# lia2790/walking-controllers

Measured on AMD Instinct MI355X. Metric: QP solves/sec (whole node), iCub IK-QP + DCM-MPC batch at 1/2/4/8 MI355X, higher is better.
Workload: dtype f64

## Files before the change

walking-controllers_amd/csrc/ik4.hip:

```cpp
#include "ik4_device.h"

namespace {

template <bool TICK, int JSRC, bool LOG = false, bool EXT = false>
__global__ __launch_bounds__(64, WCQP_IK4_WAVES)
void ik4_kernel(const IkDeviceParams* __restrict__ prm, int batch,
                const double* __restrict__ JL, const double* __restrict__ JR,
                const double* __restrict__ JN, const double* __restrict__ JC,
                const double* qpos, const double* __restrict__ state,
                double* __restrict__ dq_out, int* __restrict__ status_out,
                unsigned* __restrict__ alo_out, unsigned* __restrict__ aup_out,
                double* __restrict__ ferr_out, int* __restrict__ iters_out, const wcqp_tick::TickDev* __restrict__ tdp, int phase, int n_inner, int skip_last_mpc)
{
    __shared__ __attribute__((aligned(16))) double smem[4][PER_INST];
    if constexpr (TICK) {
        __shared__ __attribute__((aligned(16))) double kmodel[JSRC == 2 ? wcqp_tick::kKinTabSize : 2];
        __shared__ __attribute__((aligned(16))) double kgains[JSRC == 2 ? 4 * wcqp_tick::kGainsLdsStages : 2];
        ik4_tick_walk<JSRC, LOG, EXT, false>(prm, batch, JL, JR, JN, JC, qpos, state, dq_out, status_out, alo_out, aup_out, ferr_out, iters_out,
                                             tdp, phase, n_inner, skip_last_mpc, smem, kmodel, kgains);
    } else {
        ik4_body<TICK, JSRC>(prm, batch, JL, JR, JN, JC, qpos, state, dq_out, status_out, alo_out, aup_out, ferr_out, iters_out, wcqp_tick::TickDev{}, smem, xcd_group((int)blockIdx.x, (int)gridDim.x));
    }
}

// ... 1 lines not shown
__global__ __launch_bounds__(64)
void tick_mpc_prime_kernel(wcqp_tick::TickDev td, int t)
{
    __shared__ __attribute__((aligned(16))) double s_hull[4][WCQP_HULL_ROWS][4];
    const int lane = threadIdx.x, grp = lane >> 4, j = lane & 15;
    const long inst_raw = (long)blockIdx.x * 4 + grp;
    const bool live = inst_raw < td.batch;
    const long inst = live ? inst_raw : (long)td.batch - 1;
    wcqp_tick::TickMpcRegs mreg;
    wcqp_tick::tick_mpc_issue(td, j, inst, t, mreg);
    wcqp_tick::tick_mpc_finish<false, EXT>(td, j, inst, live, t, mreg, s_hull[grp]);
}


__global__ __launch_bounds__(64, WCQP_IK4_WAVES)
void qp_pair_kernel(const IkDeviceParams* __restrict__ prm, int batch,
                    const double* __restrict__ JL, const double* __restrict__ JR,
                    const double* __restrict__ JN, const double* __restrict__ JC,
                    const double* qpos, const double* __restrict__ state,
                    double* __restrict__ dq_out, int* __restrict__ status_out,
                    unsigned* __restrict__ alo_out, unsigned* __restrict__ aup_out,
                    double* __restrict__ ferr_out, int* __restrict__ iters_out, int ik_blocks, MpcPairArgs m)
{
    __shared__ __attribute__((aligned(16))) double smem[4][PER_INST];
    const bool is_mpc = (int)blockIdx.x >= ik_blocks;
    const int blk = is_mpc ? (int)blockIdx.x - ik_blocks : xcd_group((int)blockIdx.x, ik_blocks);
    if (is_mpc) {
        static_assert(wcqp_mpc::kInstPerWave * WCQP_HULL_ROWS * 4 <= 4 * PER_INST, "the hull rows fit the IK's LDS");
        double (*s_hull)[WCQP_HULL_ROWS][4] = reinterpret_cast<double (*)[WCQP_HULL_ROWS][4]>(&smem[0][0]);
        const int lane = threadIdx.x;
        const int sub = lane / wcqp_mpc::kLanesPerInstance, t = lane % wcqp_mpc::kLanesPerInstance;
        const long inst_raw = (long)blk * wcqp_mpc::kInstPerWave + sub;
        const bool live = inst_raw < batch;
        const long inst = live ? inst_raw : (long)batch - 1;
        const double2* rp = reinterpret_cast<const double2*>(m.ref) + inst * m.ref_len;
        double ux, uy, margin;
        int st;
        unsigned mask;
        wcqp_mpc::mpc_row_solve(m.c, t, inst, m.x0, rp, m.ref_len, m.u_prev, m.hull_A, m.hull_b, m.hull_nc, inst, s_hull[sub], ux, uy, st, mask, margin);
        if (t == 0 && live) {
            reinterpret_cast<double2*>(m.u0)[inst] = make_double2(ux, uy);
            m.status[inst] = st;
            if (m.active) m.active[inst] = mask;
            if (m.margin) m.margin[inst] = margin;
        }
        return;
    }
    ik4_body<false>(prm, batch, JL, JR, JN, JC, qpos, state, dq_out, status_out, alo_out, aup_out, ferr_out, iters_out, wcqp_tick::TickDev{}, smem, blk);
}

template <bool WITH_MPC>
__device__ __forceinline__
void plan_walk(const IkDeviceParams* __restrict__ prm, int batch, const wcqp_qp_step* __restrict__ recs, int n_steps, int ways, int groups,
               const wcqp_mpc::MpcDeviceConsts& c, unsigned* queue, double (*smem)[PER_INST])
{
    const bool dynamic = ways == 0;
    unsigned z = threadIdx.x;
    __asm__ volatile("" : "+v"(z));
    z >>= 6;
    constexpr unsigned QS = wcqp_ik::kPlanQueueStride / 4u;
    const unsigned total = (unsigned)n_steps * (unsigned)groups;
    unsigned home = blockIdx.x % wcqp_ik::kPlanQueues;
    auto draw = [&]() -> unsigned {
#ifndef WCQP_PLAN_STEAL
#define WCQP_PLAN_STEAL (wcqp_ik::kPlanQueues - 1u)
#endif
        for (unsigned tried = 0; tried <= WCQP_PLAN_STEAL; ++tried) {
            unsigned k = 0;
            if (threadIdx.x == 0) k = __hip_atomic_fetch_add(queue + home * QS + z, 1u, __ATOMIC_RELAXED, __HIP_MEMORY_SCOPE_AGENT);
            const unsigned u = (unsigned)__builtin_amdgcn_readfirstlane((int)k) * wcqp_ik::kPlanQueues + home;
            if (u < total) return u;
            home = (home + 1u) % wcqp_ik::kPlanQueues;
        }
        return total;
    };
    int r = (int)blockIdx.x / groups, blk = (int)blockIdx.x % groups;
#ifndef WCQP_PLAN_NO_XCD_MAP
    if ((groups & 7) == 0) {
        const int n = groups >> 3, x = (int)blockIdx.x & 7, k = (int)blockIdx.x >> 3;
        r = k / n; blk = x * n + k % n;
    }
#endif
    if (dynamic) {
        const unsigned u = draw();
        r = u < total ? (int)(u % (unsigned)n_steps) : n_steps; blk = u < total ? (int)(u / (unsigned)n_steps) : 0;
    }
#pragma unroll 1
    while (r < n_steps) {
        __asm__ volatile("" ::: "memory");
        using wcqp::as_global;
        const wcqp_qp_step& s = recs[r];
        MpcPairArgs m{c, WITH_MPC ? as_global(s.x0) : nullptr, WITH_MPC ? as_global(s.ref) : nullptr, s.ref_len, WITH_MPC ? as_global(s.u_prev) : nullptr,
                      WITH_MPC ? as_global(s.hull_A) : nullptr, WITH_MPC ? as_global(s.hull_b) : nullptr, WITH_MPC ? as_global(s.hull_nc) : nullptr,
                      WITH_MPC ? as_global(s.u0) : nullptr, WITH_MPC ? as_global(s.mpc_status) : nullptr, WITH_MPC ? as_global(s.mpc_active) : nullptr,
                      WITH_MPC ? as_global(s.mpc_margin) : nullptr,
                      dynamic ? queue + home * QS + z : nullptr, 0u, WITH_MPC};
        ik4_body<false, 0, true>(prm, batch, as_global(s.J_left), as_global(s.J_right), as_global(s.J_neck), as_global(s.J_com), as_global(s.q), as_global(s.state),
                                 as_global(s.dq), as_global(s.ik_status), as_global(s.active_lower), as_global(s.active_upper),
                                 as_global(s.foot_err), as_global(s.iters), wcqp_tick::TickDev{}, smem, blk, 0, true, nullptr, nullptr, &m);
        wcqp::wave_lds_fence();
        if (dynamic) {
            unsigned u = (unsigned)__builtin_amdgcn_readfirstlane((int)m.ticket) * wcqp_ik::kPlanQueues + home;
            if (u >= total) { home = (home + 1u) % wcqp_ik::kPlanQueues; u = draw(); }
            r = u < total ? (int)(u % (unsigned)n_steps) : n_steps; blk = u < total ? (int)(u / (unsigned)n_steps) : 0;
        } else {
            r += ways;
        }
    }
    if (dynamic && threadIdx.x == 0) {
        __threadfence();
        if (atomicAdd(queue + wcqp_ik::kPlanQueues * QS, 1u) == gridDim.x - 1) {
            for (unsigned q = 0; q <= wcqp_ik::kPlanQueues; ++q) queue[q * QS] = 0u;
        }
    }
}

__global__ __launch_bounds__(64, WCQP_IK4_WAVES)
void qp_plan_kernel(const IkDeviceParams* __restrict__ prm, int batch, const wcqp_qp_step* __restrict__ recs, int n_steps, int ways, int groups,
                    wcqp_mpc::MpcDeviceConsts c, unsigned* queue)
{
    __shared__ __attribute__((aligned(16))) double smem[4][PER_INST];
    plan_walk<true>(prm, batch, recs, n_steps, ways, groups, c, queue, smem);
}
__global__ __launch_bounds__(64, WCQP_IK4_WAVES) WCQP_IK_PLAN_REGS
void ik_plan_kernel(const IkDeviceParams* __restrict__ prm, int batch, const wcqp_qp_step* __restrict__ recs, int n_steps, int ways, int groups,
                    wcqp_mpc::MpcDeviceConsts c, unsigned* queue)
{
    __shared__ __attribute__((aligned(16))) double smem[4][PER_INST];
    plan_walk<false>(prm, batch, recs, n_steps, ways, groups, c, queue, smem);
}

}

namespace wcqp_ik {

int ik4_plan_queue_grid(int batch, int n_steps) {
    int dev = 0, cus = 0;
    if (hipGetDevice(&dev) != hipSuccess || hipDeviceGetAttribute(&cus, hipDeviceAttributeMultiprocessorCount, dev) != hipSuccess || cus < 1) return -1;
    const long long total = (long long)((batch + 3) / 4) * n_steps, slots = (long long)cus * 4 * WCQP_IK4_WAVES;
    return (int)(total < slots ? total : slots);
}

int ik4_launch_plan(const IkDeviceParams* d_prm, int batch, const wcqp_qp_step* d_recs, int n_steps, int ways,
                    const wcqp_mpc::MpcDeviceConsts& c, hipStream_t stream, unsigned* d_queue, int queue_grid, bool ik_only) {
    if (!d_prm || !d_recs || batch < 1 || n_steps < 1 || ways < 0 || (ways == 0 && (!d_queue || queue_grid < 1))) return WCQP_E_INVALID;
    const int groups = (batch + 3) / 4;
    if ((long long)groups * n_steps >= (1ll << 31)) return WCQP_E_INVALID;
    const unsigned grid = ways == 0 ? (unsigned)queue_grid : (unsigned)(groups * ways);
    if (ik_only) hipLaunchKernelGGL(ik_plan_kernel, dim3(grid), dim3(64), 0, stream, d_prm, batch, d_recs, n_steps, ways, groups, c, d_queue);
    else hipLaunchKernelGGL(qp_plan_kernel, dim3(grid), dim3(64), 0, stream, d_prm, batch, d_recs, n_steps, ways, groups, c, d_queue);
    WCQP_HIP_TRY(hipGetLastError());
    return WCQP_OK;
}

int ik4_launch_pair(const IkDeviceParams* d_prm, int batch, const IkIo& io,
                    const wcqp_mpc::MpcDeviceConsts& c, const double* x0, const double* ref, int ref_len, const double* u_prev,
                    const double* hull_A, const double* hull_b, const int* hull_nc,
                    double* u0, int* mstatus, unsigned* mactive, double* mmargin, hipStream_t stream) {
    const int ik_blocks = (batch + 3) / 4;
    const int mpc_blocks = (batch + wcqp_mpc::kInstPerWave - 1) / wcqp_mpc::kInstPerWave;
    MpcPairArgs m{c, x0, ref, ref_len, u_prev, hull_A, hull_b, hull_nc, u0, mstatus, mactive, mmargin};
    hipLaunchKernelGGL(qp_pair_kernel, dim3((unsigned)(ik_blocks + mpc_blocks)), dim3(64), 0, stream, d_prm, batch,
                       io.JL, io.JR, io.JN, io.JC, io.q, io.state, io.dq, io.status, io.alo, io.aup, io.ferr, io.iters, ik_blocks, m);
    WCQP_HIP_TRY(hipGetLastError());
    return WCQP_OK;
}

template <bool TICK, int JSRC, bool LOG = false, bool EXT = false>
static void ik4_launch_as(const IkDeviceParams* prm, int batch, const IkIo& io, const wcqp_tick::TickDev* td_dev, int phase,
                          int n_inner, int skip_last_mpc, hipStream_t stream) {
    hipLaunchKernelGGL((ik4_kernel<TICK, JSRC, LOG, EXT>), dim3((unsigned)((batch + 3) / 4)), dim3(64), 0, stream, prm, batch,
                       io.JL, io.JR, io.JN, io.JC, io.q, io.state, io.dq, io.status, io.alo, io.aup, io.ferr, io.iters,
                       td_dev, phase, n_inner, skip_last_mpc);
}

int ik4_launch(const IkDeviceParams* d_prm, int batch, const IkIo& io, hipStream_t stream) {
    ik4_launch_as<false, 0>(d_prm, batch, io, nullptr, 0, 1, 0, stream);
    WCQP_HIP_TRY(hipGetLastError());
    return WCQP_OK;
}

static int tick_check(const wcqp_tick::TickDevPL& td, const TickVariant& v) {
// ... 38 lines not shown
```

walking-controllers_amd/csrc/ik4_device.h:

```cpp
#pragma once
#include <cmath>
#include <limits>
#include <type_traits>
#include "ik_common.h"
#include "tick_device.h"
#include "kin_device.h"

namespace {

using namespace wcqp_ik;

typedef double v4d __attribute__((ext_vector_type(4)));

constexpr int NR = 12;
constexpr int NROWS_IN = 18;
constexpr int KMAX = kDof - 9;
constexpr int LDC = 14;

constexpr int OFF_ST = 0;
constexpr int OFF_BV = 112;
constexpr int OFF_DB = 130;
constexpr int OFF_CT = 0;
constexpr int OFF_PB = 0;
constexpr int A_SIZE = 340;
constexpr int OFF_COL = A_SIZE;
constexpr int OFF_YV = A_SIZE + 32;
constexpr int OFF_DV = A_SIZE + 48;
constexpr int OFF_YPV = A_SIZE;
constexpr int OFF_RV = A_SIZE + 16;
constexpr int OFF_CV = A_SIZE + 32;
constexpr int OFF_ROWB = A_SIZE + 48;
constexpr int PER_INST = 440;
constexpr int K_FS = 14, K_TW = 0, K_FRB = 322, K_FR = 358;
constexpr int K_MS = 394, K_MH = 410;
constexpr int K_PF = 434;
__host__ __device__ constexpr int k_sd(int m) { return K_TW + (16 + (m >> 1)) * K_FS + 12 + (m & 1); }
static_assert(K_MH + 24 <= K_PF && K_PF < PER_INST, "the flags stash is clear of the others");
static_assert(kDof * K_FS <= K_FRB && K_FR + 36 <= K_MS && K_MH + 24 <= PER_INST && k_sd(11) < kDof * K_FS && k_sd(0) >= 32 * 4, "kinematics scratch fits; the prefix sums [32][4] stay clear of the anchor pose");
static_assert(OFF_CT + 24 * LDC + 2 <= A_SIZE && OFF_DB + 18 <= A_SIZE && OFF_PB + 12 * 18 <= A_SIZE, "LDS overlays");
static_assert(OFF_ROWB + 16 <= PER_INST && OFF_DV + 16 <= PER_INST && (PER_INST % 32 == 24 || PER_INST % 32 == 8), "instances 16 banks apart");
static_assert(KMAX <= 24, "one slot index per C^T row");
static_assert(PER_INST * 8 * 4 * 11 <= 160 * 1024, "11 blocks per CU");

#ifndef WCQP_IK4_WAVES
#define WCQP_IK4_WAVES 2
#endif
#ifdef WCQP_IK_PLAN_VGPR_HALF
#define WCQP_IK_PLAN_REGS __attribute__((amdgpu_num_vgpr(WCQP_IK_PLAN_VGPR_HALF)))
#else
#define WCQP_IK_PLAN_REGS
#endif
#ifndef WCQP_IK4_KS
#define WCQP_IK4_KS 4
#endif

#if defined(WCQP_TICK_KSTAMPS)
#define WCQP_STAMP_AT(k) do { if constexpr (TICK) { unsigned long long t__; asm volatile("s_memtime %0\n\ts_waitcnt lgkmcnt(0)" : "=s"(t__) :: "memory"); \
                              if (lane == 0 && td.stamps) td.stamps[(size_t)blk * 16 + (k)] = t__; } } while (0)
#define WCQP_STAMP(k) do { if constexpr ((k) == 0 || (k) == 12 || (k) == 14) WCQP_STAMP_AT(k); } while (0)
#define WCQP_KSTAMP(k) WCQP_STAMP_AT(k)
#elif defined(WCQP_TICK_STAMPS)
#define WCQP_STAMP(k) do { if constexpr (TICK) { unsigned long long t__; asm volatile("s_memtime %0\n\ts_waitcnt lgkmcnt(0)" : "=s"(t__) :: "memory"); \
                           if (lane == 0 && td.stamps) td.stamps[(size_t)blk * 16 + (k)] = t__; } } while (0)
#elif defined(WCQP_IK_STAMPS)
#define WCQP_STAMP(k) do { unsigned long long t__; asm volatile("s_memtime %0\n\ts_waitcnt lgkmcnt(0)" : "=s"(t__) :: "memory"); \
                           if (lane == __ffsll((long long)__ballot(true)) - 1) reinterpret_cast<unsigned long long*>(ferr_out)[(size_t)blockIdx.x * 16 + (k)] = t__; } while (0)
#else
#define WCQP_STAMP(k) do { } while (0)
#endif
#ifndef WCQP_KSTAMP
#define WCQP_KSTAMP(k) do { } while (0)
#endif

__device__ __forceinline__ void swap32(double& a, double& b) {
    const auto l = __builtin_amdgcn_permlane32_swap((unsigned)__double2loint(a), (unsigned)__double2loint(b), false, false);
    const auto h = __builtin_amdgcn_permlane32_swap((unsigned)__double2hiint(a), (unsigned)__double2hiint(b), false, false);
    a = __hiloint2double((int)h[0], (int)l[0]); b = __hiloint2double((int)h[1], (int)l[1]);
}
__device__ __forceinline__ void swap16(double& a, double& b) {
    const auto l = __builtin_amdgcn_permlane16_swap((unsigned)__double2loint(a), (unsigned)__double2loint(b), false, false);
    const auto h = __builtin_amdgcn_permlane16_swap((unsigned)__double2hiint(a), (unsigned)__double2hiint(b), false, false);
    a = __hiloint2double((int)h[0], (int)l[0]); b = __hiloint2double((int)h[1], (int)l[1]);
}

using wcqp_kin::st2;
using wcqp_kin::ld2;

struct MpcPairArgs {
    wcqp_mpc::MpcDeviceConsts c;
    const double* x0; const double* ref; int ref_len; const double* u_prev;
    const double* hull_A; const double* hull_b; const int* hull_nc;
    double* u0; int* status; unsigned* active; double* margin;
    unsigned* ticket_from = nullptr; unsigned ticket = 0;
    bool has_mpc = true;
};

template <bool TICK, int JSRC = 0, bool PAIR = false, bool LOG = false, bool EXT = false, bool REACT = false, bool GS = false, bool PL = false>
__device__ __forceinline__
void ik4_body(const IkDeviceParams* __restrict__ prm, int batch,
                const double* __restrict__ JL, const double* __restrict__ JR,
                const double* __restrict__ JN, const double* __restrict__ JC,
                const double* qpos, const double* __restrict__ state,
                double* __restrict__ dq_out, int* __restrict__ status_out,
                unsigned* __restrict__ alo_out, unsigned* __restrict__ aup_out,
                double* __restrict__ ferr_out, int* __restrict__ iters_out, const wcqp_tick::TickDev& td, double (*smem)[PER_INST], int blk,
                const int tick_now = 0, const bool do_mpc = true, const double* kmodel = nullptr, const double* gr_lds = nullptr,
                MpcPairArgs* pm = nullptr, double* carry = nullptr, int* gait = nullptr, const unsigned long long* noise_base = nullptr)
{
    static_assert(!(TICK && PAIR), "the tick kernel carries its own MPC chain");
    static_assert(TICK || !REACT, "the reactive controller is a tick form");
    static_assert(TICK || !GS, "gain scheduling is a tick form");
    static_assert(!PL || (TICK && JSRC == 2 && !LOG), "planned / streamed trajectories: the fused-kinematics tick without logger rows");
    constexpr bool ST = PL && EXT;
    constexpr bool COMPACT = JSRC == 1;
    constexpr bool KINF = JSRC == 2;
    int lane_id = threadIdx.x;
    if constexpr (TICK || PAIR) __asm__ volatile("" : "+v"(lane_id));
    const int lane = lane_id;
    const int grp = lane >> 4;
    const int j = lane & 15;
    const long inst_raw = (long)blk * 4 + grp;
    const bool live = inst_raw < batch;
    const long inst = live ? inst_raw : (long)batch - 1;
    using wcqp::at32;
    const unsigned iu = (unsigned)inst, j8 = (unsigned)j * 8u;
    double* S = smem[grp];
    double* st = S + OFF_ST;
    const double inf = std::numeric_limits<double>::infinity();
    const bool var1 = j < kDof - 16;
    const bool rhs1 = j == kDof - 16;
    const bool base1 = j >= 8 && j < 14;
    const int col1 = j + 16;

    unsigned prev_lo = 0u, prev_up = 0u;
    bool stopped = false;
    auto load_previous_set = [&]() {
        if (td.hot_start && alo_out && aup_out) { prev_lo = *at32(alo_out, iu * 4u); prev_up = *at32(aup_out, iu * 4u); }
        stopped = wcqp_tick::tick_robot_stopped(td, (int)inst);
        if (stopped) { prev_lo = 0u; prev_up = 0u; }
    };
    if constexpr (TICK && JSRC != 2) load_previous_set();

    WCQP_STAMP(0);
    const int v0i = 6 + j, v1i = var1 ? 22 + j : 0;
    double sd0, sd1, isd0, isd1, kq0, kq1, qreg0, qreg1;
    auto load_lane_constants = [&]() {
        sd0 = prm->sd[j]; sd1 = prm->sd[col1]; isd0 = prm->isd[j]; isd1 = prm->isd[col1];
        kq0 = prm->kq[v0i]; kq1 = prm->kq[v1i]; qreg0 = prm->qreg[v0i]; qreg1 = prm->qreg[v1i];
    };
    if constexpr (!KINF) load_lane_constants();
    double a0[NROWS_IN], a1[NROWS_IN];
    double q0, q1;
    double qm0, qm1;
    bool osqp_form;
    double k_pos_foot, k_att_foot, k_pos_com, kap;
    int fast_ok;
    wcqp_tick::TickMpcRegs mreg;
    double2 p_xs = make_double2(0.0, 0.0), p_up = make_double2(0.0, 0.0);
    if constexpr (PAIR) {
        if (pm->has_mpc) {
        wcqp_mpc::mpc_window_loads(pm->c, j, reinterpret_cast<const double2*>(pm->ref), iu * (unsigned)pm->ref_len, pm->ref_len, mreg.L);
        if (j == 0) { p_xs = *at32(reinterpret_cast<const double2*>(pm->x0), iu * 16u); p_up = *at32(reinterpret_cast<const double2*>(pm->u_prev), iu * 16u); }
        mreg.nc = *at32(pm->hull_nc, iu * 4u);
        mreg.ha = make_double2(0.0, 0.0); mreg.hb = 0.0;
        if (j < WCQP_HULL_ROWS) {
            mreg.ha = *at32(reinterpret_cast<const double2*>(pm->hull_A), (iu * WCQP_HULL_ROWS + (unsigned)j) * 16u);
            mreg.hb = *at32(pm->hull_b, iu * (WCQP_HULL_ROWS * 8u) + j8);
        }
        }
    }
    if constexpr (TICK && !REACT) { if (do_mpc) wcqp_tick::tick_mpc_issue<KINF>(td, j, inst, tick_now + 1, mreg); else mreg.phase0 = td.phase0[inst]; }
    double2 cr0[5], cr1[5], cdv[5];
    int ckind0 = 0, ckind1 = 0;
    double m_ux = 0.0, m_uy = 0.0;
    double2 m_r0 = make_double2(0.0, 0.0);
    double2 m_rd = make_double2(0.0, 0.0);
    if constexpr (TICK && REACT) { if (do_mpc) wcqp_tick::tick_react_issue(td, j, inst, tick_now + 1, mreg, m_r0, m_rd); else mreg.phase0 = td.phase0[inst]; }
    wcqp_tick::ZmpRegs zreg{};
    double m_s = 0.0;
    auto gsd = [&]() -> const wcqp_tick::TickDevGS& { return static_cast<const wcqp_tick::TickDevGS&>(td); };
    auto pld = [&]() -> const wcqp_tick::TickDevPL& { return static_cast<const wcqp_tick::TickDevPL&>(td); };
    double m_pf = 0.0;
    if constexpr (PL) { if (do_mpc) m_pf = wcqp_tick::plan_flags_issue<ST>(pld(), j, inst, tick_now + 1); }
    if constexpr (TICK && GS) {
        if (do_mpc) {
            wcqp_tick::zmp_state_issue(gsd(), inst, zreg);
            if constexpr (!REACT) m_rd = wcqp_tick::zmp_vel_issue(td, inst, tick_now + 1);
        }
    }
    {
        const unsigned so = iu * (unsigned)(kStateLen * 8);
        const double* sp = at32(state, so + j8);
        const double* sp5 = at32(state, so + 640u + (j < kStateLen - 80 ? j8 : 0u));
        double sreg[6];
        double2 p_r01 = make_double2(0.0, 0.0);
        double p_r2 = 0.0;
        if constexpr (!KINF) {
#pragma unroll
            for (int m = 0; m < 5; ++m) sreg[m] = sp[m * 16];
// ... 121 lines not shown
            load_lane_constants();
            load_handoff();
            load_previous_set();
            load_measured_joints();
            wcqp::wave_lds_fence();
            if (j >= 11 && j < 14) {
                double* db = S + OFF_DB;
                const int cm = j - 11;
                const double e0 = cm == 0 ? 1.0 : 0.0, e1 = cm == 1 ? 1.0 : 0.0, e2 = cm == 2 ? 1.0 : 0.0;
                double Bc[3][3];
#pragma unroll
                for (int f = 0; f < 3; ++f) {
                    const double d0 = kdv[3 * f], d1 = kdv[3 * f + 1], d2 = kdv[3 * f + 2];
                    Bc[f][0] = e1 * d2 - e2 * d1; Bc[f][1] = e2 * d0 - e0 * d2; Bc[f][2] = e0 * d1 - e1 * d0;
                }
#pragma unroll
                for (int r = 0; r < 3; ++r) { db[r * 3 + cm] = Bc[1][r] - Bc[0][r]; db[9 + r * 3 + cm] = Bc[2][r] - Bc[0][r]; }
            }
            if (do_mpc) {
                if (j < 2) {
                    const double* ms = S + K_MS + j * 8;
                    mreg.s01 = ld2(ms); mreg.s23 = ld2(ms + 2); mreg.s45 = ld2(ms + 4); mreg.s67 = ld2(ms + 6);
                }
                if (!REACT && j < 8) { const double* mh = S + K_MH + j * 3; mreg.ha.x = mh[0]; mreg.ha.y = mh[1]; mreg.hb = mh[2]; }
            }
        } else if constexpr (COMPACT) {
            const double* jb = td.jcomp + inst * td.cstride;
            const int off0 = wcqp_tick::compact_offset(td.cmaskL, td.cmaskR, td.cmaskN, j, ckind0);
            const int off1 = wcqp_tick::compact_offset(td.cmaskL, td.cmaskR, td.cmaskN, var1 ? col1 : 0, ckind1);
#pragma unroll
            for (int m = 0; m < 5; ++m) { cr0[m] = ld2(jb + off0 + 2 * m); cr1[m] = ld2(jb + off1 + 2 * m); }
#pragma unroll
            for (int m = 0; m < 5; ++m) cdv[m] = ld2(jb + td.coff_d + 2 * m);
        } else {
        const int fc0 = 6 + j;
        const int fc1 = var1 ? 22 + j : (base1 ? j - 8 : 0);
        const unsigned o6 = iu * (unsigned)(6 * kNV * 8), o3 = iu * (unsigned)(3 * kNV * 8), c0b = (unsigned)fc0 * 8u, c1b = (unsigned)fc1 * 8u;
        const double* jl0 = at32(JL, o6 + c0b), *jl1 = at32(JL, o6 + c1b);
        const double* jr0 = at32(JR, o6 + c0b), *jr1 = at32(JR, o6 + c1b);
        const double* jc0 = at32(JC, o3 + c0b), *jc1 = at32(JC, o3 + c1b);
        const double* jn0 = at32(JN, o3 + c0b), *jn1 = at32(JN, o3 + c1b);
#pragma unroll
        for (int r = 0; r < 6; ++r) { a0[r] = jl0[r * kNV]; a1[r] = jl1[r * kNV]; }
#pragma unroll
        for (int r = 0; r < 6; ++r) { a0[6 + r] = jr0[r * kNV]; a1[6 + r] = jr1[r * kNV]; }
#pragma unroll
        for (int r = 0; r < 3; ++r) { a0[12 + r] = jc0[r * kNV]; a1[12 + r] = jc1[r * kNV]; }
#pragma unroll
        for (int r = 0; r < 3; ++r) { a0[15 + r] = jn0[r * kNV]; a1[15 + r] = jn1[r * kNV]; }
        }
        __builtin_amdgcn_sched_barrier(0);
        if constexpr (PAIR) {
            if (pm->ticket_from && threadIdx.x == 0) pm->ticket = __hip_atomic_fetch_add(pm->ticket_from, 1u, __ATOMIC_RELAXED, __HIP_MEMORY_SCOPE_AGENT);
            __builtin_amdgcn_sched_barrier(0);
        }
        if constexpr (PAIR) if (pm->has_mpc) {
            double ux, uy, u0x, u0y, margin;
            int mst_;
            unsigned mact;
            wcqp_mpc::mpc_row_partial(pm->c, j, mreg.L, ux, uy);
            if (pm->c.N >= 4 * wcqp_mpc::kLanesPerInstance)
                wcqp_mpc::mpc_row_extra_passes(pm->c, j, reinterpret_cast<const double2*>(pm->ref) + inst * pm->ref_len, pm->ref_len, ux, uy);
            if (j == 0) wcqp_mpc::mpc_row_add_state(pm->c, p_xs, p_up, ux, uy);
            wcqp_mpc::mpc_row_finish(pm->c, j, ux, uy, mreg.nc, mreg.ha.x, mreg.ha.y, mreg.hb, reinterpret_cast<double (*)[4]>(S + OFF_COL), u0x, u0y, mst_, mact, margin);
            if (j == 0 && live) {
                *at32(reinterpret_cast<double2*>(pm->u0), iu * 16u) = make_double2(u0x, u0y);
                *at32(pm->status, iu * 4u) = mst_;
                if (pm->active) *at32(pm->active, iu * 4u) = mact;
                if (pm->margin) *at32(pm->margin, iu * 8u) = margin;
            }
        }
        if constexpr (TICK) {
            double2 kg = make_double2(0.0, 0.0);
            if constexpr (GS) {
                if (do_mpc) {
                    if constexpr (!KINF) m_s = wcqp_tick::zmp_smoother_advance(gsd(), inst, j == 0 && live, m_rd, zreg);
                    kg = wcqp_tick::zmp_gains_at(td, gsd().zg, m_s);
                }
            }
            if constexpr (REACT) {
                if (do_mpc) {
                    if constexpr (!KINF) m_ux = wcqp_tick::tick_react_law(td, j, mreg, m_r0, m_rd);
                    wcqp_tick::tick_react_finish<EXT, GS>(td, j, inst, live, tick_now + 1, mreg, m_r0, m_ux, noise_base, kg);
                }
            } else if (do_mpc) {
                int code1;
                if constexpr (PL) code1 = wcqp_tick::plan_code((int)S[K_PF]);
                else {
                    const int cyc1 = *gait + 1 == 2 * td.step_ticks ? 0 : *gait + 1;
                    code1 = wcqp_tick::contact_code_cyc(cyc1, td.step_ticks, td.ds_ticks);
                }
                if constexpr (KINF) wcqp_tick::tick_mpc_finish_from<false, GS, PL, ST>(td, j, inst, live, tick_now + 1, mreg, m_r0, m_ux, m_uy, reinterpret_cast<double (*)[4]>(S + K_MS), code1, noise_base, kg);
                else wcqp_tick::tick_mpc_finish<false, false, GS>(td, j, inst, live, tick_now + 1, mreg, reinterpret_cast<double (*)[4]>(S + OFF_COL), nullptr, code1, noise_base, kg);
            }
            if (!PL && j < 6) {
                const int code = wcqp_tick::contact_code_cyc(*gait, td.step_ticks, td.ds_ticks);
                const double tw = g_sw * wcqp_tick::swing_profile_cyc(td, *gait);
                g_twl = (code == 0 || code == 2) ? 0.0 : tw;
                g_twr = (code == 1 || code == 2) ? 0.0 : tw;
            }
            if (live && j == 0 && g_ok == 0.0) td.mpc_fail[inst] += 1;
            WCQP_STAMP(13);
        }
        osqp_form = prm->form == WCQP_IK_FORM_OSQP;
        k_pos_foot = prm->k_pos_foot; k_att_foot = prm->k_att_foot; k_pos_com = prm->k_pos_com;
        kap = prm->kappa * (-prm->k_neck);
// ... 34 lines not shown
    wcqp::wave_lds_fence();
    if constexpr (LOG) {
        if (tick_now < td.logger_ticks && live) {
            double* row = td.log_rows + ((size_t)tick_now * td.batch + inst) * wcqp_tick::kLoggerCols;
            if (j < 2) {
                const double* hd = td.hand + ((size_t)(tick_now & 1) * td.batch + inst) * wcqp_tick::kHandLen;
                const double r0 = td.ref_traj[((size_t)inst * td.traj_len + tick_now) * 2 + j];
                const double r1 = td.ref_traj[((size_t)inst * td.traj_len + tick_now + 1) * 2 + j];
                row[j] = hd[6 + j]; row[2 + j] = r0; row[4 + j] = (r1 - r0) / td.dT;
                if constexpr (REACT) row[4 + j] = td.dcm_vel[((size_t)inst * td.traj_len + tick_now) * 2 + j];
                row[6 + j] = hd[10 + j]; row[8 + j] = hd[12 + j];
                row[13 + j] = hd[j]; row[15 + j] = hd[2 + j];
            }
            if (j < 3) {
                row[10 + j] = st[66 + j];
                row[17 + j] = st[j]; row[23 + j] = st[12 + j]; row[29 + j] = st[24 + j]; row[35 + j] = st[36 + j];
            }
            if (j < 4) {
                const double* R = st + (j == 0 ? 3 : (j == 1 ? 15 : (j == 2 ? 27 : 39)));
                double* o = row + (j == 0 ? 20 : (j == 1 ? 26 : (j == 2 ? 32 : 38)));
                const double s_ = fmin(1.0, fmax(-1.0, -R[6]));
                o[0] = atan2(R[7], R[8]); o[1] = asin(s_); o[2] = atan2(R[3], R[0]);
            }
        }
    }
    if constexpr (COMPACT) {
        auto unpack = [&](const double2 (&r)[5], int kind, double (&a)[NROWS_IN]) {
            const double x[6] = {r[1].y, r[2].x, r[2].y, r[3].x, r[3].y, r[4].x};
            const double mL = kind == 1 ? 1.0 : 0.0, mR = kind == 2 ? 1.0 : 0.0, mN = kind == 3 ? 1.0 : 0.0;
#pragma unroll
            for (int r_ = 0; r_ < 6; ++r_) { a[r_] = mL * x[r_]; a[6 + r_] = mR * x[r_]; }
            a[12] = r[0].x; a[13] = r[0].y; a[14] = r[1].x;
#pragma unroll
            for (int r_ = 0; r_ < 3; ++r_) a[15 + r_] = mN * x[r_];
        };
        unpack(cr0, ckind0, a0);
        unpack(cr1, ckind1, a1);
        if (!var1) {
#pragma unroll
            for (int r_ = 0; r_ < NROWS_IN; ++r_) a1[r_] = 0.0;
        }
    }
#ifdef WCQP_IK4_EXIT_AFTER_LOADS
    {
        double acc = q0 + q1 + st[j];
#pragma unroll
        for (int r = 0; r < NROWS_IN; ++r) acc += a0[r] + a1[r];
        if (live) dq_out[inst * kDof + j] = acc + sd0 + sd1 + isd0 + isd1 + kq0 + kq1 + qreg0 + qreg1 + (double)fast_ok + k_pos_foot + k_att_foot + k_pos_com + kap + (osqp_form ? 1.0 : 0.0);
        return;
    }
#endif

    WCQP_STAMP(1);
    double b_mine = 0.0;
    {
        double* bv = S + OFF_BV;
        if (j < 15) {
            if (j < 12) {
                const int foot = j / 6, k = j % 6;
                const double* p  = st + (foot ? 12 : 0);
                const double* R  = st + (foot ? 15 : 3);
                const double* pd = st + (foot ? 36 : 24);
                const double* Rd = st + (foot ? 39 : 27);
                const double* tw = st + (foot ? 81 : 75);
                const double corr = k < 3 ? k_pos_foot * (p[k] - pd[k]) : k_att_foot * rot_err(R, Rd, k - 3);
                const bool skip = osqp_form && tw[0] == tw[1] && tw[0] == 0.0;
                b_mine = skip ? tw[k] : tw[k] - corr;
            } else {
                const int k = j - 12;
                b_mine = st[72 + k] - k_pos_com * (st[66 + k] - st[69 + k]);
            }
            bv[j] = b_mine;
        }
        if (j >= 13) bv[15 + (j - 13)] = kap * rot_err(st + 48, st + 57, j - 13);
    }
    if constexpr (!EXT) { qm0 = q0; qm1 = q1; }
    const double gt0 = -sd0 * kq0 * (qreg0 - qm0);
    const double gt1 = var1 ? -sd1 * kq1 * (qreg1 - qm1) : 0.0;
    wcqp::wave_lds_fence();
    if (rhs1) {
        const double* bv = S + OFF_BV;
#pragma unroll
        for (int r = 0; r < NROWS_IN; r += 2) { const double2 b2 = ld2(bv + r); a1[r] = b2.x; a1[r + 1] = b2.y; }
    }

    WCQP_STAMP(2);
    bool pat = true;
    if constexpr (KINF) {
    } else if constexpr (COMPACT) {
        double* db = S + OFF_DB;
        if (j >= 11 && j < 14) {
            const int cm = j - 11;
            const double e0 = cm == 0 ? 1.0 : 0.0, e1 = cm == 1 ? 1.0 : 0.0, e2 = cm == 2 ? 1.0 : 0.0;
            double Bc[3][3];
#pragma unroll
            for (int f = 0; f < 3; ++f) {
                const double d0 = f == 0 ? cdv[0].x : (f == 1 ? cdv[1].y : cdv[3].x);
                const double d1 = f == 0 ? cdv[0].y : (f == 1 ? cdv[2].x : cdv[3].y);
                const double d2 = f == 0 ? cdv[1].x : (f == 1 ? cdv[2].y : cdv[4].x);
                Bc[f][0] = e1 * d2 - e2 * d1; Bc[f][1] = e2 * d0 - e0 * d2; Bc[f][2] = e0 * d1 - e1 * d0;
            }
#pragma unroll
            for (int r = 0; r < 3; ++r) { db[r * 3 + cm] = Bc[1][r] - Bc[0][r]; db[9 + r * 3 + cm] = Bc[2][r] - Bc[0][r]; }
        }
    } else {
        double* db = S + OFF_DB;
// ... 62 lines not shown
            for (int r = 0; r < NR; r += 2) st2(c + r, rhs1 ? 0.0 : c1[r], rhs1 ? 0.0 : c1[r + 1]);
            st2(c + NR, gt1, 0.0);
        }
        if (rhs1) {
#pragma unroll
            for (int r = 0; r < NR; r += 2) st2(dv + r, c1[r], c1[r + 1]);
            ct[24 * LDC] = 0.0; ct[24 * LDC + 1] = 0.0;
        }
    }
    wcqp::wave_lds_fence();
    WCQP_STAMP(10);
    {
        const int mk = lane & 15, mq = lane >> 4;
        v4d acc[4];
#pragma unroll
        for (int g = 0; g < 4; ++g) acc[g] = v4d{0.0, 0.0, 0.0, 0.0};
#pragma unroll
        for (int s = 0; s < 6; ++s) {
#pragma unroll
            for (int g = 0; g < 4; ++g) {
                const double v = smem[g][OFF_CT + (4 * s + mq) * LDC + mk];
                acc[g] = __builtin_amdgcn_mfma_f64_16x16x4f64(v, v, acc[g], 0, 0, 0);
            }
        }
        WCQP_STAMP(11);
        double t[4][4];
#pragma unroll
        for (int reg = 0; reg < 4; ++reg) {
            double x0 = acc[0][reg], x1 = acc[1][reg], x2 = acc[2][reg], x3 = acc[3][reg];
            swap32(x0, x2); swap32(x1, x3);
            swap16(x0, x1); swap16(x2, x3);
            t[0][reg] = x0; t[1][reg] = x1; t[2][reg] = x2; t[3][reg] = x3;
        }
        const double* dv = S + OFF_DV;
        const bool rowok = j < NR, is12 = j == NR;
        const double dj = dv[j < NR ? j : 0];
        const double sgn = rowok ? 1.0 : (is12 ? -1.0 : 0.0), m12 = is12 ? 1.0 : 0.0, mrow = rowok ? -1.0 : 0.0;
#pragma unroll
        for (int k = 0; k < NR; k += 2) {
            const double2 d2 = ld2(dv + k);
            const double h0 = t[k & 3][k >> 2], h1 = t[(k + 1) & 3][(k + 1) >> 2];
            double v0 = fma(m12, d2.x, h0), v1 = fma(m12, d2.y, h1);
            if (k < 3) v0 += (k == j) ? 1.0 : 0.0;
            if (k + 1 < 3) v1 += (k + 1 == j) ? 1.0 : 0.0;
            Hr[k] = sgn * v0;
            Hr[k + 1] = sgn * v1;
        }
        Hr[NR] = mrow * (t[NR & 3][NR >> 2] + dj);
    }

    WCQP_STAMP(5);
    const double tol = prm->tol;
    const int max_iter = prm->max_iter;
    double lo0 = prm->vlo[v0i] * isd0, hi0 = prm->vhi[v0i] * isd0, lo1 = prm->vlo[v1i] * isd1, hi1 = prm->vhi[v1i] * isd1;
    bool ok = true;
    {
        double* col = S + OFF_COL;
        static_assert(OFF_DV + 16 == OFF_COL + 64, "the column pairs take the 64 doubles of region B");
        double pmin = 1.0;
        col[j] = Hr[0];
        col[16 + j] = Hr[1];
        wcqp::wave_lds_fence();
#pragma unroll
        for (int k = 0; k < NR; k += 2) {
            const int buf = (k >> 1) & 1;
            const double* cA = col + 32 * buf;
            const double* cB = cA + 16;
            double ca[NR + 2], cb2[NR + 2];
#pragma unroll
            for (int q = 0; q <= NR; q += 2) {
                const double2 x2 = ld2(cA + q), y2 = ld2(cB + q);
                ca[q] = x2.x; ca[q + 1] = x2.y; cb2[q] = y2.x; cb2[q + 1] = y2.y;
            }
            const double pa = ca[k], pb = ca[k + 1], pd = cb2[k + 1];
            const double det = fma(pa, pd, -pb * pb);
            pmin = (pa > 0.0 && det > 0.0) ? pmin : -1.0;
            const double idet = wcqp::fast_rcp(det);
            const double i11 = pd * idet, i12 = -pb * idet, i22 = pa * idet;
            const double m1 = Hr[k], m2 = Hr[k + 1];
            const double g1 = fma(m1, i11, m2 * i12), g2 = fma(m1, i12, m2 * i22);
            const double ek = (j == k) ? 1.0 : 0.0, ek1 = (j == k + 1) ? 1.0 : 0.0;
            const double f1 = fma(-ek1, i12, fma(-ek, i11, g1));
            const double f2 = fma(-ek1, i22, fma(-ek, i12, g2));
            if (k + 2 < NR) {
                Hr[k + 2] = fma(-f2, cb2[k + 2], fma(-f1, ca[k + 2], Hr[k + 2]));
                Hr[k + 3] = fma(-f2, cb2[k + 3], fma(-f1, ca[k + 3], Hr[k + 3]));
                double* nb = col + 32 * (buf ^ 1);
                nb[j] = Hr[k + 2];
                nb[16 + j] = Hr[k + 3];
            }
#pragma unroll
            for (int q = 0; q <= NR; ++q) {
                if (q == k || q == k + 1) continue;
                if (k + 2 < NR && (q == k + 2 || q == k + 3)) continue;
                Hr[q] = fma(-f2, cb2[q], fma(-f1, ca[q], Hr[q]));
            }
            Hr[k] = f1 - ek;
            Hr[k + 1] = f2 - ek1;
#pragma unroll
            for (int q = 0; q <= NR; ++q) __asm__ volatile("" : "+v"(Hr[q]));
            wcqp::wave_lds_fence();
        }
        ok = pmin > 0.0;
    }
    WCQP_STAMP(6);
    const double* ct0 = S + OFF_CT + j * LDC;
    const double* ct1 = S + OFF_CT + (var1 ? col1 : 23) * LDC;
    double nu0, nu1;
    {
        double* yv = S + OFF_YV;
        yv[j] = j < NR ? Hr[NR] : 0.0;
        wcqp::wave_lds_fence();
        double s0 = gt0, s1 = gt1;
#pragma unroll
        for (int r = 0; r < NR; r += 2) {
            const double2 y2 = ld2(yv + r);
            const double2 a2 = ld2(ct0 + r), b2 = ld2(ct1 + r);
            s0 = fma(a2.x, y2.x, s0); s0 = fma(a2.y, y2.y, s0);
            s1 = fma(b2.x, y2.x, s1); s1 = fma(b2.y, y2.y, s1);
        }
        nu0 = -s0;
        nu1 = var1 ? -s1 : 0.0;
    }
    wcqp::wave_lds_fence();

    WCQP_STAMP(7);
    int st_code = ok ? WCQP_STATUS_SOLVED : WCQP_STATUS_NUMERIC;
    int it = 0;
    bool in_w0 = false, in_w1 = false;
    double sig0 = 0.0, sig1 = 0.0;
    const bool bnd1 = var1;
    lo1 = bnd1 ? lo1 : -inf; hi1 = bnd1 ? hi1 : inf;
    const bool need = !stopped && !osqp_form && (fmax(nu0 - hi0, lo0 - nu0) > tol || (bnd1 && fmax(nu1 - hi1, lo1 - nu1) > tol));
    const unsigned long long need_m = __ballot(need);
    if (((need_m >> (16 * grp)) & 0xffffull) != 0ull && st_code == WCQP_STATUS_SOLVED) {
        double* ypv = S + OFF_YPV;
        double* rvec = S + OFF_RV;
        double* cvec = S + OFF_CV;
        double* rowb = S + OFF_ROWB;
        auto Wi = [&](int a) -> int& { return *reinterpret_cast<int*>(S + OFF_CT + a * LDC + 13); };
        const int rowbase = lane & 48;
        bool pending = false;
        int p = 0;
        double sig = 0.0, s = 0.0, tp0 = 0.0, tp1 = 0.0, ppp = 1.0, mu_p = 0.0;
        bool done = false;
        int nW = 0;
        constexpr int KS = WCQP_IK4_KS;
        double Rs[KS][KS], sgS[KS], muS[KS], tvS[KS], tc0[KS], tc1[KS];
        int wS[KS];
#pragma unroll
        for (int a = 0; a < KS; ++a) {
            sgS[a] = 0.0; muS[a] = 0.0; tvS[a] = 0.0; wS[a] = 0; tc0[a] = 0.0; tc1[a] = 0.0;
#pragma unroll
            for (int b = 0; b < KS; ++b) Rs[a][b] = 0.0;
        }
        auto most_violated = [&]() -> unsigned {
            const double viol0 = !in_w0 ? fmax(nu0 - hi0, lo0 - nu0) : -inf;
            const double viol1 = (bnd1 && !in_w1) ? fmax(nu1 - hi1, lo1 - nu1) : -inf;
// ... 373 lines not shown
                                const double2 r2 = ld2(rvec + b);
                                const double u0 = me ? -r2.x * inz : fma(ra_inz, r2.x, myR[b]);
                                const double u1 = me ? -r2.y * inz : fma(ra_inz, r2.y, myR[b + 1]);
                                myR[b] = (b == n) ? (me ? inz : -ra_inz) : u0;
                                myR[b + 1] = (b + 1 == n) ? (me ? inz : -ra_inz) : u1;
                            }
                            if (me) { s_live = true; s_var = p; s_sg = sig; s_mu = mu_p; Wi(n) = p; }
                            if (p == j) { in_w0 = true; sig0 = sig; slot0 = n; }
                            if (p == col1) { in_w1 = true; sig1 = sig; slot1 = n; }
                            ++nW;
                            pending = false;
                        } else {
                            const unsigned dm = (unsigned)((__ballot(ratio == t1) >> (16 * grp)) & 0xffffull);
                            const int jd = dm ? __ffs(dm) - 1 : 0;
                            wcqp::wave_lds_fence();
                            if (j == jd) {
#pragma unroll
                                for (int b = 0; b < KMAX; b += 2) st2(rowb + b, myR[b], myR[b + 1]);
                            }
                            wcqp::wave_lds_fence();
                            const int wdrop = Wi(jd);
                            double myjd = 0.0;
                            const double djj = rowb[jd];
                            myjd = rowb[j < KMAX ? j : 0];
                            const double f = (s_live && j != jd) ? myjd * wcqp::fast_rcp(djj) : 0.0;
#pragma unroll
                            for (int b = 0; b < KMAX; b += 2) {
                                const double2 d2 = ld2(rowb + b);
                                myR[b] = (j == jd || b == jd) ? 0.0 : fma(-f, d2.x, myR[b]);
                                myR[b + 1] = (j == jd || b + 1 == jd) ? 0.0 : fma(-f, d2.y, myR[b + 1]);
                            }
                            if (j == jd) { s_live = false; s_mu = 0.0; }
                            if (wdrop == j) { in_w0 = false; sig0 = 0.0; }
                            if (wdrop == col1) { in_w1 = false; sig1 = 0.0; }
                            --nW;
                            ++it;
                        }
                    }
                }
                wcqp::wave_lds_fence();
            }
        }
        {
            const double d0 = in_w0 ? fabs(nu0 - (sig0 > 0.0 ? hi0 : lo0)) : fmax(nu0 - hi0, lo0 - nu0);
            const double d1 = !bnd1 ? 0.0 : (in_w1 ? fabs(nu1 - (sig1 > 0.0 ? hi1 : lo1)) : fmax(nu1 - hi1, lo1 - nu1));
            const double dev = fmax(d0 == d0 ? d0 : inf, d1 == d1 ? d1 : inf);
            const unsigned bad = row_max_u32((dev > 1e-9) ? 1u : 0u);
            if (st_code == WCQP_STATUS_SOLVED && bad != 0u) st_code = WCQP_STATUS_NUMERIC;
        }
    }

    WCQP_STAMP(8);
    double dq0 = nu0 * sd0, dq1 = nu1 * sd1;
    if (st_code == WCQP_STATUS_SOLVED && in_w0) dq0 = sig0 > 0.0 ? prm->vhi[v0i] : prm->vlo[v0i];
    if (st_code == WCQP_STATUS_SOLVED && in_w1) dq1 = sig1 > 0.0 ? prm->vhi[v1i] : prm->vlo[v1i];
    const bool nonfinite = row_max_u32((isfinite(dq0) && (!var1 || isfinite(dq1))) ? 0u : 1u) != 0u;
    if (nonfinite) { st_code = WCQP_STATUS_NUMERIC; dq0 = 0.0; dq1 = 0.0; in_w0 = false; in_w1 = false; }
    const unsigned long long bu0 = __ballot(in_w0 && sig0 > 0.0), bu1 = __ballot(in_w1 && sig1 > 0.0);
    const unsigned long long bl0 = __ballot(in_w0 && sig0 < 0.0), bl1 = __ballot(in_w1 && sig1 < 0.0);
    if (!use) {
        st_code = WCQP_STATUS_STRUCTURE;
        dq0 = 0.0; dq1 = 0.0;
    }
    if (live) {
        double* dqo = at32(dq_out, iu * (unsigned)(kDof * 8) + j8);
        dqo[0] = dq0;
        if (var1) dqo[16] = dq1;
        if (j == 0) {
            const unsigned up = (unsigned)((bu0 >> (16 * grp)) & 0xffffull) | ((unsigned)((bu1 >> (16 * grp)) & 0x7full) << 16);
            const unsigned dn = (unsigned)((bl0 >> (16 * grp)) & 0xffffull) | ((unsigned)((bl1 >> (16 * grp)) & 0x7full) << 16);
            *at32(status_out, iu * 4u) = st_code;
            if (aup_out) *at32(aup_out, iu * 4u) = use ? up : 0u;
            if (alo_out) *at32(alo_out, iu * 4u) = use ? dn : 0u;
            if (iters_out) *at32(iters_out, iu * 4u) = it;
        }
    }
#ifdef WCQP_IK_STAMPS
    WCQP_STAMP(9);
    return;
#endif
    if constexpr (TICK) {
        const bool ik_ok = st_code == WCQP_STATUS_SOLVED;
        if (live) {
            const int i_ = (int)inst;
            const double v0 = (ik_ok && !stopped) ? dq0 : 0.0, v1 = (ik_ok && !stopped) ? dq1 : 0.0;
            carry[0] += 0.5 * td.dT * (v0 + carry[2]); carry[2] = v0;
            const size_t g0 = (size_t)i_ * kDof + j;
            double* qd = at32(td.q_des.get(), iu * (unsigned)(kDof * 8) + j8), *dp = at32(td.dq_prev.get(), iu * (unsigned)(kDof * 8) + j8);
            qd[0] = carry[0]; dp[0] = v0;
            if (tick_now < td.log_ticks) td.dq_log[(size_t)tick_now * td.batch * kDof + g0] = v0;
            if (var1) {
                carry[1] += 0.5 * td.dT * (v1 + carry[3]); carry[3] = v1;
                const size_t g1 = (size_t)i_ * kDof + col1;
                qd[16] = carry[1]; dp[16] = v1;
                if (tick_now < td.log_ticks) td.dq_log[(size_t)tick_now * td.batch * kDof + g1] = v1;
            }
            if (j == 0 && (!ik_ok || stopped)) td.ik_fail[i_] += 1;
        }
        if constexpr (PL) { if (do_mpc) *gait = (int)S[K_PF]; }
        WCQP_STAMP(14);
    }
    if (ferr_out) {
        double* pb = S + OFF_PB;
        double* uv = S + OFF_YV;
        const int fc0 = 6 + j, fc1 = var1 ? 22 + j : 6;
        const double v1 = var1 ? dq1 : 0.0;
        const double* jl = JL + inst * (6 * kNV);
        const double* jr = JR + inst * (6 * kNV);
        double part[12];
#pragma unroll
        for (int r = 0; r < 6; ++r) {
            part[r] = fma(jl[r * kNV + fc0], dq0, jl[r * kNV + fc1] * v1);
            part[6 + r] = fma(jr[r * kNV + fc0], dq0, jr[r * kNV + fc1] * v1);
        }
        wcqp::wave_lds_fence();
#pragma unroll
        for (int r = 0; r < 12; ++r) pb[r * 18 + j] = part[r];
        wcqp::wave_lds_fence();
        double u_mine = 0.0;
        if (j < 12) {
            u_mine = b_mine;
#pragma unroll
            for (int k = 0; k < 16; k += 2) { const double2 p2 = ld2(pb + j * 18 + k); u_mine -= p2.x; u_mine -= p2.y; }
            uv[j] = u_mine;
        }
        wcqp::wave_lds_fence();
        if (j < 12 && live && use) {
            const int rr = j % 6, foot = j / 6;
            const double wa0 = uv[3], wa1 = uv[4], wa2 = uv[5];
            double jv;
            if (rr < 3) {
                const double* bl = jl + rr * kNV + 3;
// ... 121 lines not shown
```

Measured before the change: 1.192 billion.

## Prefetch next plan record pointers and stage per-DOF tables in LDS

```diff
diff --git a/walking-controllers_amd/csrc/ik4.hip b/walking-controllers_amd/csrc/ik4.hip
--- a/walking-controllers_amd/csrc/ik4.hip
+++ b/walking-controllers_amd/csrc/ik4.hip
@@ -77,7 +77,7 @@
 template <bool WITH_MPC>
 __device__ __forceinline__
 void plan_walk(const IkDeviceParams* __restrict__ prm, int batch, const wcqp_qp_step* __restrict__ recs, int n_steps, int ways, int groups,
-               const wcqp_mpc::MpcDeviceConsts& c, unsigned* queue, double (*smem)[PER_INST])
+               const wcqp_mpc::MpcDeviceConsts& c, unsigned* queue, double (*smem)[PER_INST], double* tab)
 {
     const bool dynamic = ways == 0;
     unsigned z = threadIdx.x;
@@ -110,19 +110,41 @@
         const unsigned u = draw();
         r = u < total ? (int)(u % (unsigned)n_steps) : n_steps; blk = u < total ? (int)(u / (unsigned)n_steps) : 0;
     }
+#ifndef WCQP_PLAN_NO_LDS_TABLES
+    plan_tables_to_lds(prm, tab);
+#else
+    tab = nullptr;
+#endif
+#ifndef WCQP_PLAN_NO_RECORD_AHEAD
+    constexpr bool kAhead = true;
+#else
+    constexpr bool kAhead = false;
+#endif
+    PlanInputs in = plan_inputs_of(recs[r < n_steps ? r : n_steps - 1]);
 #pragma unroll 1
     while (r < n_steps) {
         __asm__ volatile("" ::: "memory");
+#if defined(WCQP_PLAN_LINK_STAMPS)
+        unsigned long long t_top;
+        WCQP_LSTAMP_READ(t_top);
+#endif
         using wcqp::as_global;
         const wcqp_qp_step& s = recs[r];
-        MpcPairArgs m{c, WITH_MPC ? as_global(s.x0) : nullptr, WITH_MPC ? as_global(s.ref) : nullptr, s.ref_len, WITH_MPC ? as_global(s.u_prev) : nullptr,
-                      WITH_MPC ? as_global(s.hull_A) : nullptr, WITH_MPC ? as_global(s.hull_b) : nullptr, WITH_MPC ? as_global(s.hull_nc) : nullptr,
-                      WITH_MPC ? as_global(s.u0) : nullptr, WITH_MPC ? as_global(s.mpc_status) : nullptr, WITH_MPC ? as_global(s.mpc_active) : nullptr,
-                      WITH_MPC ? as_global(s.mpc_margin) : nullptr,
-                      dynamic ? queue + home * QS + z : nullptr, 0u, WITH_MPC};
-        ik4_body<false, 0, true>(prm, batch, as_global(s.J_left), as_global(s.J_right), as_global(s.J_neck), as_global(s.J_com), as_global(s.q), as_global(s.state),
+        if (dynamic || !kAhead) in = plan_inputs_of(s);
+        const int r_next = r + ways < n_steps ? r + ways : n_steps - 1;
+        PlanArgs m{{c, WITH_MPC ? as_global(in.x0) : nullptr, WITH_MPC ? as_global(in.ref) : nullptr, in.ref_len, WITH_MPC ? as_global(in.u_prev) : nullptr,
+                    WITH_MPC ? as_global(in.hull_A) : nullptr, WITH_MPC ? as_global(in.hull_b) : nullptr, WITH_MPC ? as_global(in.hull_nc) : nullptr,
+                    WITH_MPC ? as_global(s.u0) : nullptr, WITH_MPC ? as_global(s.mpc_status) : nullptr, WITH_MPC ? as_global(s.mpc_active) : nullptr,
+                    WITH_MPC ? as_global(s.mpc_margin) : nullptr,
+                    dynamic ? queue + home * QS + z : nullptr, 0u, WITH_MPC},
+                   kAhead ? recs + r_next : nullptr, PlanInputs{}, tab};
+#if defined(WCQP_PLAN_LINK_STAMPS)
+        m.t_top = t_top;
+#endif
+        ik4_body<false, 0, true>(prm, batch, as_global(in.JL), as_global(in.JR), as_global(in.JN), as_global(in.JC), as_global(in.q), as_global(in.state),
                                  as_global(s.dq), as_global(s.ik_status), as_global(s.active_lower), as_global(s.active_upper),
                                  as_global(s.foot_err), as_global(s.iters), wcqp_tick::TickDev{}, smem, blk, 0, true, nullptr, nullptr, &m);
+        if (kAhead) in = m.next;
         wcqp::wave_lds_fence();
         if (dynamic) {
             unsigned u = (unsigned)__builtin_amdgcn_readfirstlane((int)m.ticket) * wcqp_ik::kPlanQueues + home;
@@ -145,14 +167,16 @@
                     wcqp_mpc::MpcDeviceConsts c, unsigned* queue)
 {
     __shared__ __attribute__((aligned(16))) double smem[4][PER_INST];
-    plan_walk<true>(prm, batch, recs, n_steps, ways, groups, c, queue, smem);
+    __shared__ __attribute__((aligned(16))) double tab[PLAN_TAB_SIZE];
+    plan_walk<true>(prm, batch, recs, n_steps, ways, groups, c, queue, smem, tab);
 }
 __global__ __launch_bounds__(64, WCQP_IK4_WAVES) WCQP_IK_PLAN_REGS
 void ik_plan_kernel(const IkDeviceParams* __restrict__ prm, int batch, const wcqp_qp_step* __restrict__ recs, int n_steps, int ways, int groups,
                     wcqp_mpc::MpcDeviceConsts c, unsigned* queue)
 {
     __shared__ __attribute__((aligned(16))) double smem[4][PER_INST];
-    plan_walk<false>(prm, batch, recs, n_steps, ways, groups, c, queue, smem);
+    __shared__ __attribute__((aligned(16))) double tab[PLAN_TAB_SIZE];
+    plan_walk<false>(prm, batch, recs, n_steps, ways, groups, c, queue, smem, tab);
 }
 
 }
diff --git a/walking-controllers_amd/csrc/ik4_device.h b/walking-controllers_amd/csrc/ik4_device.h
--- a/walking-controllers_amd/csrc/ik4_device.h
+++ b/walking-controllers_amd/csrc/ik4_device.h
@@ -71,6 +71,15 @@
 #ifndef WCQP_KSTAMP
 #define WCQP_KSTAMP(k) do { } while (0)
 #endif
+#if defined(WCQP_PLAN_LINK_STAMPS)
+#define WCQP_LSTAMP_READ(t) asm volatile("s_memtime %0\n\ts_waitcnt lgkmcnt(0)" : "=s"(t) :: "memory")
+#define WCQP_LSTAMP(k) do { if constexpr (PAIR) { unsigned long long t__; WCQP_LSTAMP_READ(t__); \
+                            if (lane == 0 && ferr_out) reinterpret_cast<unsigned long long*>(ferr_out)[(size_t)blk * 48 + (k)] = t__; } } while (0)
+#define WCQP_LSTAMP_DRAIN() do { if constexpr (PAIR) asm volatile("s_waitcnt vmcnt(0)" ::: "memory"); } while (0)
+#else
+#define WCQP_LSTAMP(k) do { } while (0)
+#define WCQP_LSTAMP_DRAIN() do { } while (0)
+#endif
 
 __device__ __forceinline__ void swap32(double& a, double& b) {
     const auto l = __builtin_amdgcn_permlane32_swap((unsigned)__double2loint(a), (unsigned)__double2loint(b), false, false);
@@ -93,6 +102,40 @@
     double* u0; int* status; unsigned* active; double* margin;
     unsigned* ticket_from = nullptr; unsigned ticket = 0;
     bool has_mpc = true;
+};
+
+struct PlanInputs {
+    const double* x0; const double* ref; const double* u_prev; const double* hull_A; const double* hull_b; const int* hull_nc;
+    const double* JL; const double* JR; const double* JN; const double* JC; const double* q; const double* state;
+    int ref_len;
+};
+__device__ __forceinline__ PlanInputs plan_inputs_of(const wcqp_qp_step& s) {
+    return PlanInputs{s.x0, s.ref, s.u_prev, s.hull_A, s.hull_b, s.hull_nc, s.J_left, s.J_right, s.J_neck, s.J_com, s.q, s.state, s.ref_len};
+}
+constexpr int T_SD = 0, T_ISD = WCQP_MAX_DOF, T_KQ = 2 * WCQP_MAX_DOF, T_QREG = 3 * WCQP_MAX_DOF, T_VLO = 4 * WCQP_MAX_DOF, T_VHI = 5 * WCQP_MAX_DOF;
+constexpr int PLAN_TAB_SIZE = 6 * WCQP_MAX_DOF;
+#ifndef WCQP_PLAN_NO_LDS_TABLES
+constexpr bool kPlanLdsTables = true;
+#else
+constexpr bool kPlanLdsTables = false;
+#endif
+typedef const __attribute__((address_space(3))) double* lds_table_ptr;
+static_assert((4 * PER_INST + PLAN_TAB_SIZE) * 8 <= 20480, "a plan's workgroup stays under the 20 KB of LDS that two waves per SIMD allow");
+__device__ __forceinline__ void plan_tables_to_lds(const IkDeviceParams* __restrict__ prm, double* tab) {
+    const int t = threadIdx.x;
+    static_assert(sizeof(prm->sd) == WCQP_MAX_DOF * 8 && sizeof(prm->vhi) == WCQP_MAX_DOF * 8 && WCQP_MAX_DOF <= 64, "one lane per table entry");
+    if (t < WCQP_MAX_DOF) {
+        const double sd = prm->sd[t], isd = prm->isd[t], kq = prm->kq[t], qreg = prm->qreg[t], vlo = prm->vlo[t], vhi = prm->vhi[t];
+        tab[T_SD + t] = sd; tab[T_ISD + t] = isd; tab[T_KQ + t] = kq; tab[T_QREG + t] = qreg; tab[T_VLO + t] = vlo; tab[T_VHI + t] = vhi;
+    }
+    wcqp::wave_lds_fence();
+}
+struct PlanArgs : MpcPairArgs {
+    const wcqp_qp_step* next_from = nullptr; PlanInputs next{};
+    const double* tab = nullptr;
+#if defined(WCQP_PLAN_LINK_STAMPS)
+    unsigned long long t_top = 0;
+#endif
 };
 
 template <bool TICK, int JSRC = 0, bool PAIR = false, bool LOG = false, bool EXT = false, bool REACT = false, bool GS = false, bool PL = false>
@@ -142,9 +185,21 @@
     if constexpr (TICK && JSRC != 2) load_previous_set();
 
     WCQP_STAMP(0);
+#if defined(WCQP_PLAN_LINK_STAMPS)
+    if constexpr (PAIR) { if (lane == 0 && ferr_out) reinterpret_cast<unsigned long long*>(ferr_out)[(size_t)blk * 48] = static_cast<const PlanArgs*>(pm)->t_top; }
+#endif
+    WCQP_LSTAMP(1);
     const int v0i = 6 + j, v1i = var1 ? 22 + j : 0;
     double sd0, sd1, isd0, isd1, kq0, kq1, qreg0, qreg1;
+    constexpr bool TAB = PAIR && kPlanLdsTables;
+    lds_table_ptr ptab = nullptr;
+    if constexpr (TAB) ptab = (lds_table_ptr)static_cast<const PlanArgs*>(pm)->tab;
     auto load_lane_constants = [&]() {
+        if constexpr (TAB) {
+            sd0 = ptab[T_SD + j]; sd1 = ptab[T_SD + col1]; isd0 = ptab[T_ISD + j]; isd1 = ptab[T_ISD + col1];
+            kq0 = ptab[T_KQ + v0i]; kq1 = ptab[T_KQ + v1i]; qreg0 = ptab[T_QREG + v0i]; qreg1 = ptab[T_QREG + v1i];
+            return;
+        }
         sd0 = prm->sd[j]; sd1 = prm->sd[col1]; isd0 = prm->isd[j]; isd1 = prm->isd[col1];
         kq0 = prm->kq[v0i]; kq1 = prm->kq[v1i]; qreg0 = prm->qreg[v0i]; qreg1 = prm->qreg[v1i];
     };
@@ -372,6 +427,8 @@
         __builtin_amdgcn_sched_barrier(0);
         if constexpr (PAIR) {
             if (pm->ticket_from && threadIdx.x == 0) pm->ticket = __hip_atomic_fetch_add(pm->ticket_from, 1u, __ATOMIC_RELAXED, __HIP_MEMORY_SCOPE_AGENT);
+            PlanArgs* pa = static_cast<PlanArgs*>(pm);
+            if (pa->next_from) pa->next = plan_inputs_of(*pa->next_from);
             __builtin_amdgcn_sched_barrier(0);
         }
         if constexpr (PAIR) if (pm->has_mpc) {
@@ -512,6 +569,8 @@
 #endif
 
     WCQP_STAMP(1);
+    WCQP_LSTAMP_DRAIN();
+    WCQP_LSTAMP(2);
     double b_mine = 0.0;
     {
         double* bv = S + OFF_BV;
@@ -680,7 +739,9 @@
     WCQP_STAMP(5);
     const double tol = prm->tol;
     const int max_iter = prm->max_iter;
-    double lo0 = prm->vlo[v0i] * isd0, hi0 = prm->vhi[v0i] * isd0, lo1 = prm->vlo[v1i] * isd1, hi1 = prm->vhi[v1i] * isd1;
+    auto vlo_at = [&](int v) -> double { if constexpr (TAB) return ptab[T_VLO + v]; else return prm->vlo[v]; };
+    auto vhi_at = [&](int v) -> double { if constexpr (TAB) return ptab[T_VHI + v]; else return prm->vhi[v]; };
+    double lo0 = vlo_at(v0i) * isd0, hi0 = vhi_at(v0i) * isd0, lo1 = vlo_at(v1i) * isd1, hi1 = vhi_at(v1i) * isd1;
     bool ok = true;
     {
         double* col = S + OFF_COL;
@@ -732,6 +793,9 @@
         ok = pmin > 0.0;
     }
     WCQP_STAMP(6);
+    WCQP_LSTAMP(3);
+    WCQP_LSTAMP_DRAIN();
+    WCQP_LSTAMP(4);
     const double* ct0 = S + OFF_CT + j * LDC;
     const double* ct1 = S + OFF_CT + (var1 ? col1 : 23) * LDC;
     double nu0, nu1;
@@ -1211,8 +1275,13 @@
 
     WCQP_STAMP(8);
     double dq0 = nu0 * sd0, dq1 = nu1 * sd1;
-    if (st_code == WCQP_STATUS_SOLVED && in_w0) dq0 = sig0 > 0.0 ? prm->vhi[v0i] : prm->vlo[v0i];
-    if (st_code == WCQP_STATUS_SOLVED && in_w1) dq1 = sig1 > 0.0 ? prm->vhi[v1i] : prm->vlo[v1i];
+    WCQP_LSTAMP(5);
+    if (st_code == WCQP_STATUS_SOLVED && in_w0) dq0 = sig0 > 0.0 ? vhi_at(v0i) : vlo_at(v0i);
+    if (st_code == WCQP_STATUS_SOLVED && in_w1) dq1 = sig1 > 0.0 ? vhi_at(v1i) : vlo_at(v1i);
+#if defined(WCQP_PLAN_LINK_STAMPS)
+    if constexpr (PAIR) asm volatile("" : "+v"(dq0), "+v"(dq1) :: "memory");
+#endif
+    WCQP_LSTAMP(6);
     const bool nonfinite = row_max_u32((isfinite(dq0) && (!var1 || isfinite(dq1))) ? 0u : 1u) != 0u;
     if (nonfinite) { st_code = WCQP_STATUS_NUMERIC; dq0 = 0.0; dq1 = 0.0; in_w0 = false; in_w1 = false; }
     const unsigned long long bu0 = __ballot(in_w0 && sig0 > 0.0), bu1 = __ballot(in_w1 && sig1 > 0.0);
@@ -1237,6 +1306,9 @@
 #ifdef WCQP_IK_STAMPS
     WCQP_STAMP(9);
     return;
+#endif
+#if defined(WCQP_PLAN_LINK_STAMPS)
+    if constexpr (PAIR) { WCQP_LSTAMP(7); WCQP_LSTAMP(8); WCQP_LSTAMP(9); return; }
 #endif
     if constexpr (TICK) {
         const bool ik_ok = st_code == WCQP_STATUS_SOLVED;
```

Result: no change. 1.184 billion (-0.7%).
